# rvp-group/mad-icp

Hardware: NVIDIA H100
Metric: scans/sec (130k-pt scan vs 16-keyframe model) (higher is better)
Workload: dtype f64

## Files before the change

### mad_icp_b200/csrc/capi.cu

```cuda
#include <cooperative_groups.h>
#include <cuda_runtime.h>

#include <algorithm>
#include <cmath>
#include <cstdio>
#include <cstdlib>
#include <cstring>
#include <new>
#include <stdexcept>
#include <string>
#include <vector>

#include "../../include/madicp_b200_debug.h"
#include "ctx.hpp"
#include "device_kernels.cuh"

namespace madicp {

static thread_local std::string g_error;
void set_error(const std::string& msg) { g_error = msg; }

}

using namespace madicp;
// ... 792 lines not shown
  if (int rc = cloud_check(t, xyz_out, idx_out, fn)) return rc;
  const int64_t n = t->n_points;
  if (n == 0) return 0;
  madicp_ctx* c = t->ctx;
  MADICP_TRY
  CK(cudaSetDevice(c->device));
  if (size_t(n) > c->cap_cloud_out) {
    c->cap_cloud_out = 0;
    const size_t cap = size_t(n) + size_t(n) / 4 + 1024;
    CK(cudaHostAlloc(c->h_cloud_xyz.put(), cap * 3 * sizeof(double), cudaHostAllocMapped));
    CK(cudaHostAlloc(c->h_cloud_idx.put(), cap * sizeof(int64_t), cudaHostAllocMapped));
    c->cap_cloud_out = cap;
  }
  double* dx = nullptr;
  int64_t* di = nullptr;
  CK(cudaHostGetDevicePointer(reinterpret_cast<void**>(&dx), c->h_cloud_xyz, 0));
  CK(cudaHostGetDevicePointer(reinterpret_cast<void**>(&di), c->h_cloud_idx, 0));
  if (int rc = cloud_launch(t, X, xyz_out ? dx : nullptr, idx_out ? di : nullptr)) return rc;
  CK(cudaStreamSynchronize(c->stream));
  if (xyz_out) memcpy(xyz_out, c->h_cloud_xyz, size_t(n) * 3 * sizeof(double));
  if (idx_out) memcpy(idx_out, c->h_cloud_idx, size_t(n) * sizeof(int64_t));
  return n;
  MADICP_CATCH(fn)
}

int64_t madtree_gpu_cloud_dev(const madtree_gpu_t* t, const double X[12], double* xyz_out, int64_t* idx_out,
                              void* consumer_stream) {
  const char* fn = "madtree_gpu_cloud_dev";
  if (int rc = cloud_check(t, xyz_out, idx_out, fn)) return rc;
  madicp_ctx* c = t->ctx;
  CK(cudaSetDevice(c->device));
  if (xyz_out)
    if (int rc = madicp_check_device_ptr(c, xyz_out, 8, "madtree_gpu_cloud_dev (points)")) return rc;
  if (idx_out)
    if (int rc = madicp_check_device_ptr(c, idx_out, 8, "madtree_gpu_cloud_dev (indices)")) return rc;
  const int64_t n = t->n_points;
  if (n == 0) return 0;
  if (int rc = madicp_stream_wait(c, c->stream, consumer_stream)) return rc;
  if (int rc = cloud_launch(t, X, xyz_out, idx_out)) return rc;
  if (int rc = madicp_stream_wait(c, consumer_stream, c->stream)) return rc;
  return n;
}

int madtree_gpu_release_cloud(madtree_gpu_t* t) {
  if (!t) {
    set_error("madtree_gpu_release_cloud: null tree");
    return MADICP_ERR_INVALID;
  }
  t->cloud.reset();
  return MADICP_OK;
}

int madicp_put_keyframe_tree(madicp_ctx_t* c, int slot, const madtree_gpu_t* t, const double X[12]) {
  if (!c || !t || t->ctx != c || slot < 0 || slot >= c->max_keyframes || t->n_nodes < 1) {
    set_error("madicp_put_keyframe_tree: bad arguments (the tree must live on this context)");
    return MADICP_ERR_INVALID;
  }
  MADICP_TRY
  CK(cudaSetDevice(c->device));
  int rc = ensure_pool(c, size_t(t->n_nodes));
  if (rc) return rc;
  const double* X_dev = nullptr;
  if (X) {
    rc = stage_pose(c, X, &X_dev);
    if (rc) return rc;
  }
  CK(cudaMemcpyAsync(c->d_pool_lvl + size_t(slot) * (kMaxLevels + 1), t->lvl, size_t(t->n_levels + 1) * sizeof(int),
                     cudaMemcpyDeviceToDevice, c->stream));
  Slot& s = c->slots[slot];
  s.n_nodes = t->n_nodes;
  s.n_leaves = t->n_leaves;
  s.n_levels = t->n_levels;
  return build_slot(c, slot, t->recs, X_dev);
  MADICP_CATCH("madicp_put_keyframe_tree")
}

static int ensure_moving(madicp_ctx* c, int L) {
  if (size_t(L) <= c->cap_moving) return MADICP_OK;
  CK(cudaStreamSynchronize(c->stream));
  c->cap_moving = 0;
  const size_t cap = size_t(L) + size_t(L) / 4 + 1024;
  CK(cudaMalloc(c->d_moving.put(), cap * 3 * sizeof(double)));
  CK(cudaMalloc(c->d_mov4.put(), cap * sizeof(Moving4)));
  CK(cudaMalloc(c->d_step_matched.put(), cap));
  c->cap_moving = cap;
  return MADICP_OK;
}

static int prepare_moving(madicp_ctx* c) {
  if (!c->mov4_stale || c->L < 1) return MADICP_OK;
  k_prepare_moving<<<blocks_for(c->L), kStepBlock, 0, c->stream>>>(c->d_moving, c->L, c->P, c->d_mov4, nullptr, nullptr);
  c->launches++;
  CK(cudaGetLastError());
  c->mov4_stale = false;
  return MADICP_OK;
}

int madicp_set_moving(madicp_ctx_t* c, const double* means, int L) {
  if (!c || !means || L < 1 || size_t(L) > kMatchedCap) {
    set_error("madicp_set_moving: bad arguments (1 <= L <= 1048576)");
    return MADICP_ERR_INVALID;
  }
  CK(cudaSetDevice(c->device));
  int rc = ensure_moving(c, L);
  if (rc) return rc;
  CK(cudaMemcpyAsync(c->d_moving, means, size_t(L) * 3 * sizeof(double), cudaMemcpyHostToDevice, c->stream));
  c->L = L;
  c->mov4_stale = true;
  return prepare_moving(c);
}

int madicp_set_moving_tree(madicp_ctx_t* c, const madtree_gpu_t* t) {
  if (!c || !t || t->ctx != c || t->n_leaves < 1 || size_t(t->n_leaves) > kMatchedCap) {
    set_error("madicp_set_moving_tree: bad arguments (the tree must live on this context)");
    return MADICP_ERR_INVALID;
  }
  CK(cudaSetDevice(c->device));
  int rc = ensure_moving(c, t->n_leaves);
  if (rc) return rc;
  c->L = t->n_leaves;
  k_prepare_moving<<<blocks_for(c->L), kStepBlock, 0, c->stream>>>(c->d_moving, c->L, c->P, c->d_mov4, t->recs, t->leaf_of);
  c->launches++;
  CK(cudaGetLastError());
  c->mov4_stale = false;
  return MADICP_OK;
}

int madicp_get_moving(madicp_ctx_t* c, double* means_out, int cap) {
  if (!c || !means_out || c->L < 1 || cap < c->L) return MADICP_ERR_INVALID;
  CK(cudaSetDevice(c->device));
  CK(cudaMemcpyAsync(means_out, c->d_moving, size_t(c->L) * 3 * sizeof(double), cudaMemcpyDeviceToHost, c->stream));
  CK(cudaStreamSynchronize(c->stream));
  return c->L;
}

static int check_ready(madicp_ctx* c, const char* who) {
  if (!c) return MADICP_ERR_INVALID;
  if (c->L < 1 || !c->d_moving) {
    set_error(std::string(who) + ": no moving leaves (call madicp_set_moving first)");
    return MADICP_ERR_STATE;
  }
  if (int64_t(madicp_num_keyframes(c)) * int64_t(c->L) >= (int64_t(1) << 31)) {
    set_error(std::string(who) + ": keyframes x moving leaves must stay below 2^31 (32-bit item index)");
    return MADICP_ERR_INVALID;
  }
  if (madicp_num_keyframes(c) < 1 && c->world <= 1) {
    set_error(std::string(who) + ": no keyframe uploaded");
    return MADICP_ERR_STATE;
  }
  return MADICP_OK;
}

static int launch_search(madicp_ctx* c, const ModelView& mv, const double* d_X, bool want_ord) {
  const int64_t items = int64_t(mv.K) * c->L;
  int rc = ensure_items(c, size_t(items));
  if (rc) return rc;
  rc = prepare_moving(c);
  if (rc) return rc;
  k_search<<<grid_for(c, items), kStepBlock, 0, c->stream>>>(mv, c->d_mov4, c->L, d_X, c->d_hit,
                                                            want_ord ? c->d_ord.get() : nullptr);
  c->launches++;
  CK(cudaGetLastError());
  return MADICP_OK;
}

int madicp_search(madicp_ctx_t* c, const double X[12], int32_t* out) {
// ... 20 lines not shown
  if (rc) return rc;
  if (!X || !H || !b) return MADICP_ERR_INVALID;
  CK(cudaSetDevice(c->device));
  const ModelView mv = make_view(c);
  if (mv.K < 1) {
    set_error("madicp_linearize: no keyframe on this device");
    return MADICP_ERR_STATE;
  }
  memcpy(c->h_pinned, X, 12 * sizeof(double));
  CK(cudaMemcpyAsync(c->d_X, c->h_pinned, 12 * sizeof(double), cudaMemcpyHostToDevice, c->stream));
  rc = launch_search(c, mv, c->d_X, false);
  if (rc) return rc;
  CK(cudaMemsetAsync(c->d_state, 0, 16, c->stream));
  CK(cudaMemsetAsync(c->d_step_matched, 0, size_t(c->L), c->stream));
  const int64_t items = int64_t(mv.K) * c->L;
  const int grid = grid_for(c, items);
  k_linearize<<<grid, kStepBlock, 0, c->stream>>>(mv, c->d_mov4, c->L, c->d_X, c->P, c->d_hit, c->d_step_matched,
                                                 c->d_partial, c->d_state);
  c->launches++;
  CK(cudaGetLastError());
  CK(cudaMemcpyAsync(c->h_state, c->d_state, offsetof(GnState, X_trace), cudaMemcpyDeviceToHost, c->stream));
  if (matched) CK(cudaMemcpyAsync(c->h_matched, c->d_step_matched, size_t(c->L), cudaMemcpyDeviceToHost, c->stream));
  CK(cudaStreamSynchronize(c->stream));
  memcpy(H, c->h_state->H, sizeof(double) * 36);
  memcpy(b, c->h_state->b, sizeof(double) * 6);
  if (matched) memcpy(matched, c->h_matched, size_t(c->L));
  return MADICP_OK;
}

int madicp_solve_update(madicp_ctx_t* c, const double H[36], const double b[6], double X[12]) {
  if (!c || !H || !b || !X) return MADICP_ERR_INVALID;
  CK(cudaSetDevice(c->device));
  memcpy(c->h_pinned, X, 12 * sizeof(double));
  memcpy(c->h_pinned + 12, H, 36 * sizeof(double));
  memcpy(c->h_pinned + 48, b, 6 * sizeof(double));
  CK(cudaMemcpyAsync(c->d_X, c->h_pinned, 54 * sizeof(double), cudaMemcpyHostToDevice, c->stream));
  k_solve<<<1, 32, 0, c->stream>>>(c->d_X + 12, c->d_X + 48, c->d_X);
  c->launches++;
  CK(cudaGetLastError());
  CK(cudaMemcpyAsync(c->h_pinned, c->d_X, 12 * sizeof(double), cudaMemcpyDeviceToHost, c->stream));
  CK(cudaStreamSynchronize(c->stream));
  memcpy(X, c->h_pinned, 12 * sizeof(double));
  return MADICP_OK;
}

int madicp_debug_inv_det6(madicp_ctx_t* c, const double H[36], double* weight) {
  if (!c || !H || !weight) return MADICP_ERR_INVALID;
  CK(cudaSetDevice(c->device));
  memcpy(c->h_pinned + 12, H, 36 * sizeof(double));
  CK(cudaMemcpyAsync(c->d_X + 12, c->h_pinned + 12, 36 * sizeof(double), cudaMemcpyHostToDevice, c->stream));
  k_inv_det6<<<1, 32, 0, c->stream>>>(c->d_X + 12, c->d_X + 48);
  c->launches++;
  CK(cudaGetLastError());
  CK(cudaMemcpyAsync(c->h_pinned + 48, c->d_X + 48, sizeof(double), cudaMemcpyDeviceToHost, c->stream));
  CK(cudaStreamSynchronize(c->stream));
  *weight = c->h_pinned[48];
  return MADICP_OK;
}

static int register_enqueue(madicp_ctx* c, int iters, const double X0[12], int clear_from) {
  int rc = check_ready(c, "madicp_register");
  if (rc) return rc;
  if (!X0 || iters < 1 || iters > MADICP_MAX_ITERS) {
    set_error("madicp_register: bad arguments (1 <= iters <= 64 per launch)");
    return MADICP_ERR_INVALID;
  }
  CK(cudaSetDevice(c->device));
  rc = prepare_moving(c);
  if (rc) return rc;
  rc = pick_shape(c, int64_t(madicp_num_keyframes(c)) * c->L);
  if (rc) return rc;
  GnArgs A;
  A.model = make_view(c);
  A.P = c->P;
  A.peers.rank = c->rank;
  A.peers.world = c->world;
  A.peers.epoch_base = c->epoch;
  const int mb = int(c->call_seq & 1u);
  for (int r = 0; r < kMaxPeers; ++r) {
    A.peers.box[r] = (r < c->world) ? &c->peer_comm[r]->box : nullptr;
    A.peer_matched[r] = (r < c->world) ? c->peer_comm[r]->matched[mb] : nullptr;
  }
  A.moving = c->d_mov4;
  A.L = c->L;
  A.iters = iters;
  A.clear_from = clear_from;
  A.matched = c->d_comm->matched[mb];
  size_t map_bytes = 0;
  {
    const size_t per_cta = gn_map_bytes(unsigned(madicp_num_keyframes(c)), unsigned(c->L), unsigned(c->gn_grid));
    const size_t ctas = size_t(c->gn_grid / c->sm_count);
    auto bucket = [&](size_t dynamic) {
      const size_t bytes = ctas * (dynamic + c->gn_static_smem + 1024);
      const size_t kb[] = {8, 16, 32, 64, 100, 132, 164, 196, 228};
      for (size_t b : kb)
        if (bytes <= b * 1024) return b;
      return size_t(1 << 20);
    };
    if (per_cta && bucket(c->gn_smem + per_cta) == bucket(c->gn_smem)) map_bytes = per_cta;
  }
  A.map_in_smem = map_bytes ? 1 : 0;
  {
    const size_t stride =
        ((size_t(c->max_keyframes) * gn_share_bound(c->cap_moving, unsigned(c->gn_grid))) + 31) & ~size_t(31);
    const size_t need = stride * size_t(c->gn_grid);
    if (need > c->cap_memo) {
      CK(cudaStreamSynchronize(c->stream));
      c->cap_memo = 0;
      const size_t cap = need + need / 4;
      CK(cudaMalloc(c->d_memo_leaf.put(), cap * sizeof(int)));
      CK(cudaMalloc(c->d_memo_margin.put(), cap * sizeof(float)));
      CK(cudaMalloc(c->d_memo_ckpt.put(), cap * sizeof(unsigned)));
      CK(cudaMalloc(c->d_memo_ckpt_up.put(), cap * sizeof(float)));
      c->cap_memo = cap;
    }
    A.memo_leaf = c->d_memo_leaf;
    A.memo_margin = c->d_memo_margin;
    A.memo_ckpt = c->d_memo_ckpt;
    A.memo_ckpt_up = c->d_memo_ckpt_up;
    A.item_stride = int(stride);
    A.memo_mode = c->memo_mode;
    A.walk_buf = mb;
  }
  A.st = c->d_state;
  A.dbg = c->d_dbg;
  A.dbg_cta = c->d_dbg ? c->d_dbg_cta.get() : nullptr;
  c->epoch += uint32_t(iters);
  A.pose_epoch = c->pose_epoch;
  c->pose_epoch += uint32_t(iters);
  memcpy(A.X0, X0, 12 * sizeof(double));
  A.tiles = c->d_tiles;
  A.zero_next = c->d_comm->matched[mb ^ 1];
  A.zero_bytes = int((std::min(kMatchedCap, c->cap_moving) + 15) & ~size_t(15));
  void* args[] = {&A};
  CK(cudaLaunchCooperativeKernel(c->gn_kernel, dim3(c->gn_grid), dim3(c->gn_threads), args, c->gn_smem + map_bytes, c->stream));
  c->launches++;
  c->last_iters = iters;
  c->call_seq++;
  return MADICP_OK;
}

int madicp_register_async(madicp_ctx_t* c, int iters, const double X0[12]) {
  return register_enqueue(c, iters, X0, iters - 1);
}
int madicp_register_partial_async(madicp_ctx_t* c, int iters, const double X0[12]) {
  return register_enqueue(c, iters, X0, 0);
}

int madicp_register_fetch_weight(madicp_ctx_t* c, double X[12], double H[36], double b[6], uint8_t* matched, int* n_matched,
                                 double* weight) {
  if (!c || c->last_iters < 1) {
    set_error("madicp_register_fetch: nothing was enqueued");
    return MADICP_ERR_STATE;
  }
  CK(cudaSetDevice(c->device));
  CK(cudaMemcpyAsync(c->h_state, c->d_state, offsetof(GnState, X_trace), cudaMemcpyDeviceToHost, c->stream));
  if (matched)
    CK(cudaMemcpyAsync(c->h_matched, c->d_comm->matched[(c->call_seq - 1u) & 1u], size_t(c->L), cudaMemcpyDeviceToHost,
                       c->stream));
  CK(cudaStreamSynchronize(c->stream));
  if (c->h_state->error) {
    set_error("madicp_register: a peer GPU never delivered its H/b tile (rank down, or no matching registration enqueued there)");
    CK(cudaMemsetAsync(&c->d_state->error, 0, sizeof(int), c->stream));
    return MADICP_ERR_COMM;
  }
  if (X) memcpy(X, c->h_state->X_out, 12 * sizeof(double));
  if (H) memcpy(H, c->h_state->H, 36 * sizeof(double));
  if (b) memcpy(b, c->h_state->b, 6 * sizeof(double));
  if (matched) memcpy(matched, c->h_matched, size_t(c->L));
  if (n_matched) *n_matched = c->h_state->n_matched;
  if (weight) *weight = c->h_state->weight;
  return MADICP_OK;
}
int madicp_register_fetch(madicp_ctx_t* c, double X[12], double H[36], double b[6], uint8_t* matched, int* n_matched) {
  return madicp_register_fetch_weight(c, X, H, b, matched, n_matched, nullptr);
}

int madicp_register(madicp_ctx_t* c, int iters, double X[12], double H[36], double b[6], uint8_t* matched,
                    int* n_matched) {
  if (!c || !X || iters < 0) {
    set_error("madicp_register: bad arguments");
    return MADICP_ERR_INVALID;
  }
  if (iters == 0) {
    if (H) memset(H, 0, 36 * sizeof(double));
    if (b) memset(b, 0, 6 * sizeof(double));
    if (matched && c->L > 0) memset(matched, 0, size_t(c->L));
    if (n_matched) *n_matched = 0;
    return MADICP_OK;
  }
  int left = iters;
  while (left > MADICP_MAX_ITERS) {
    int rc = register_enqueue(c, MADICP_MAX_ITERS, X, MADICP_MAX_ITERS);
    if (rc) return rc;
    rc = madicp_register_fetch(c, X, nullptr, nullptr, nullptr, nullptr);
    if (rc) return rc;
    left -= MADICP_MAX_ITERS;
  }
  int rc = register_enqueue(c, left, X, left - 1);
  if (rc) return rc;
  return madicp_register_fetch(c, X, H, b, matched, n_matched);
}
// ... 271 lines not shown
```

### mad_icp_b200/csrc/ctx.hpp

```cpp
#pragma once
#include <cuda_runtime.h>

#include <atomic>
#include <memory>
#include <mutex>
#include <new>
#include <stdexcept>
#include <string>
#include <vector>

#include "cuda_owned.hpp"
#include "kernels.cuh"

namespace madicp {
void set_error(const std::string& msg);

constexpr int kMaxLevels = 4096;
struct Slot {
  int n_nodes = 0, n_leaves = 0, n_levels = 0;
};
constexpr size_t kMatchedCap = size_t(1) << 20;

struct CommBlock {
  Mailbox box;
  unsigned char matched[2][kMatchedCap];
};

struct CloudBuf {
  size_t cap = 0;
  DevPtr<double> xyz;
  DevPtr<int32_t> idx;
};
}

struct madicp_ctx;

struct madtree_gpu {
  madicp_ctx* ctx = nullptr;
  madtree_rec_t* recs = nullptr;
  int* lvl = nullptr;
  int* leaf_of = nullptr;
  size_t cap_nodes = 0;
  void* block = nullptr;
  int n_nodes = 0, n_leaves = 0, n_levels = 0;
  std::vector<int> h_lvl;
  double* full = nullptr;
  int64_t n_points = 0;
  uint64_t build_seq = 0;
  std::shared_ptr<madicp::CloudBuf> cloud;
  int64_t cloud_off = 0;
};

struct madicp_ctx {
  ~madicp_ctx();
  int device = 0;
  int max_keyframes = 0;
  madicp::Stream own_stream;
  cudaStream_t stream = nullptr;
  int sm_count = 0;
  std::vector<madicp::Slot> slots;
  size_t pool_cap = 0;
  madicp::DevPtr<madtree_rec_t> d_pool_recs;
  madicp::DevPtr<int> d_pool_child0;
  madicp::DevPtr<int> d_pool_rec_of;
  madicp::DevPtr<int> d_pool_lvl;
  size_t quad_cap = 0;
  madicp::DevPtr<madicp::QuadRec> d_quad;
  madicp::DevPtr<double> d_pool_ww;
  static constexpr int kXformRing = 64;
  madicp::DevPtr<double> d_xform;
  madicp::HostPtr<double> h_xform;
  madicp::HostPtr<int> h_lvl;
  madicp::Event xform_done[kXformRing];
  uint32_t xform_seq = 0;
  static constexpr int kGatherRing = 8;
  madicp::HostPtr<madicp::LeafGather> h_gather;
  madicp::DevPtr<madicp::LeafGather> d_gather;
  size_t cap_gather = 0;
  madicp::Event gather_done[kGatherRing];
  uint32_t gather_seq = 0;
  madicp::DevPtr<double> d_leaves;
  madicp::HostPtr<double> h_leaves;
  size_t cap_leaves = 0;
  std::vector<madtree_gpu*> tree_cache;
  std::vector<madicp::DevPtr<void>> tree_slabs;
  madicp::Event tree_free_ev;
  madicp::Event xstream_ev;
  std::mutex tree_mu;
  bool keep_cloud = false;
  std::vector<madicp::CloudBuf*> cloud_cache;
  std::mutex cloud_mu;
  madicp::HostPtr<int64_t> h_cloud_idx;
  madicp::HostPtr<double> h_cloud_xyz;
  size_t cap_cloud_out = 0;
  void* build_state = nullptr;
  void* plan_state = nullptr;
  madicp::DevPtr<long long> d_dbg_cta;
  madicp::IcpParams P{0.2, 0.31622776601683794, 0.02};
  madicp::DevPtr<double> d_moving;
  madicp::DevPtr<madicp::Moving4> d_mov4;
  bool mov4_stale = true;
  madicp::DevPtr<unsigned char> d_step_matched;
  int L = 0;
  size_t cap_moving = 0;
  uint32_t call_seq = 0;
  madicp::DevPtr<int> d_hit;
  madicp::DevPtr<int> d_ord;
  size_t cap_items = 0;
  madicp::DevPtr<double> d_cloud_q;
  madicp::DevPtr<int> d_cloud_o;
  size_t cap_cloud = 0;
  madicp::DevPtr<double> d_partial;
  madicp::DevPtr<madicp::LLCell> d_tiles;
  size_t cap_partial = 0;
  madicp::DevPtr<int> d_memo_leaf;
  madicp::DevPtr<float> d_memo_margin;
  madicp::DevPtr<unsigned> d_memo_ckpt;
  madicp::DevPtr<float> d_memo_ckpt_up;
  size_t cap_memo = 0;
  int memo_mode = 2;
  madicp::DevPtr<madicp::GnState> d_state;
  madicp::DevPtr<double> d_X;
  madicp::DevPtr<madicp::CommBlock> d_comm;
  madicp::HostPtr<double> h_pinned;
  madicp::HostPtr<madicp::GnState> h_state;
  madicp::HostPtr<unsigned char> h_matched;
  int gn_grid = 0;
  bool gn_auto = true;
  int gn_threads = 1024;
  const void* gn_kernel = nullptr;
  size_t gn_smem = 0;
  size_t gn_static_smem = 0;
  static constexpr int kNumAutoShapes = 5;
  static constexpr int kAutoShapes[kNumAutoShapes] = {768, 896, 704, 640, 512};
  double pass_cost[kNumAutoShapes] = {4935.0, 6195.0, 5060.0, 4925.0, 4165.0};
  bool calibrated = false;
  int last_iters = 0;
  madicp::DevPtr<long long> d_dbg;
  std::atomic<int64_t> launches{0};
  int rank = 0, world = 1;
  madicp::CommBlock* peer_comm[madicp::kMaxPeers] = {};
  uint32_t epoch = 0;
  uint32_t pose_epoch = 1;
};

#define CK(call)                                                                                   \
  do {                                                                                             \
    cudaError_t e_ = (call);                                                                       \
    if (e_ != cudaSuccess) {                                                                       \
      madicp::set_error(std::string(#call) + ": " + cudaGetErrorString(e_));                       \
      return MADICP_ERR_CUDA;                                                                      \
    }                                                                                              \
  } while (0)

#define MADICP_TRY try {
#define MADICP_CATCH(who)                                          \
  }                                                                \
  catch (const std::bad_alloc&) {                                  \
    madicp::set_error(std::string(who) + ": out of host memory");  \
    return MADICP_ERR_NOMEM;                                       \
  }                                                                \
  catch (const std::exception& e_) {                               \
    madicp::set_error(std::string(who) + ": " + e_.what());        \
    return MADICP_ERR_INVALID;                                     \
  }

int madicp_tree_alloc(madicp_ctx* c, size_t cap_nodes, madtree_gpu** out);
int madicp_cloud_alloc(madicp_ctx* c, size_t n, std::shared_ptr<madicp::CloudBuf>* out);
int madicp_check_device_ptr(madicp_ctx* c, const void* p, int align, const char* fn);
int madicp_stream_wait(madicp_ctx* c, void* waiter, void* signaller);
void madicp_gpu_build_release(madicp_ctx* c);
```

### mad_icp_b200/csrc/device_kernels.cuh

```cuda
#pragma once
#include "gn_partition.h"
#include "kernels.cuh"

namespace madicp {


__device__ __forceinline__ int depth_of(const int* __restrict__ lvl, int n_levels, int i) {
  int lo = 0, hi = n_levels;
  while (hi - lo > 1) {
    const int mid = (lo + hi) >> 1;
    if (__ldg(lvl + mid) <= i) lo = mid; else hi = mid;
  }
  return lo;
}

__global__ void __launch_bounds__(kStepBlock)
k_slot_ingest(const madtree_rec_t* src, madtree_rec_t* dst, int n, const double* __restrict__ Xp,
              const int* __restrict__ lvl, int n_levels, int* __restrict__ flag) {
  const int i = blockIdx.x * kStepBlock + threadIdx.x;
  if (i >= n) return;
  Rec r = load_rec_plain(src + i);
  const int npts = src[i].num_points;
  int f = 0;
  if (r.link >= 0 && (depth_of(lvl, n_levels, i) & 1) == 0)
// ... 277 lines not shown
  }
}

__global__ void __launch_bounds__(kStepBlock)
k_search_cloud(const __grid_constant__ ModelView model, int root, const char* __restrict__ q, int64_t n, int64_t q_stride,
               int q_is_f32, int* __restrict__ ordinals, double* __restrict__ points, double* __restrict__ normals,
               double* __restrict__ dists) {
  for (int64_t i = int64_t(blockIdx.x) * kStepBlock + threadIdx.x; i < n; i += int64_t(gridDim.x) * kStepBlock) {
    const char* r = q + i * q_stride;
    double qx, qy, qz;
    if (q_is_f32) {
      const float* f = reinterpret_cast<const float*>(r);
      qx = double(__ldg(f)); qy = double(__ldg(f + 1)); qz = double(__ldg(f + 2));
    } else {
      const double* d = reinterpret_cast<const double*>(r);
      qx = __ldg(d); qy = __ldg(d + 1); qz = __ldg(d + 2);
    }
    double ww;
    const Rec f = load_rec(model.recs + descend(model, root, qx, qy, qz, ww));
    if (ordinals) ordinals[i] = -1 - f.link;
    if (points) {
      points[3 * i] = f.mx; points[3 * i + 1] = f.my; points[3 * i + 2] = f.mz;
    }
    if (normals) {
      normals[3 * i] = f.dx; normals[3 * i + 1] = f.dy; normals[3 * i + 2] = f.dz;
    }
    if (dists) dists[i] = norm3(qx - f.mx, qy - f.my, qz - f.mz);
  }
}


template <int THREADS>
__device__ __forceinline__ void peer_allreduce(const PeerView& pv, uint32_t epoch, double* s_tot,
                                               double (*s_peer)[kAcc], int* error) {
  const int slot = int(epoch & 1u);
  for (int idx = threadIdx.x; idx < pv.world * kAcc; idx += THREADS) {
    const int r = idx / kAcc, i = idx - r * kAcc;
    const double v = s_tot[i];
    const uint32_t lo = uint32_t(__double2loint(v)), hi = uint32_t(__double2hiint(v));
    LLCell* dst = &pv.box[r]->cell[slot][pv.rank][i];
    asm volatile("st.volatile.global.v4.u32 [%0], {%1,%2,%3,%4};" ::"l"(dst), "r"(lo), "r"(epoch), "r"(hi), "r"(epoch)
                 : "memory");
  }
  for (int idx = threadIdx.x; idx < pv.world * kAcc; idx += THREADS) {
    const int r = idx / kAcc, i = idx - r * kAcc;
    const LLCell* src = &pv.box[pv.rank]->cell[slot][r][i];
    uint32_t lo, f0, hi, f1, spins = 0;
    do {
      asm volatile("ld.volatile.global.v4.u32 {%0,%1,%2,%3}, [%4];" : "=r"(lo), "=r"(f0), "=r"(hi), "=r"(f1) : "l"(src)
                   : "memory");
      if (++spins == (1u << 26)) {
        *error = 1;
        break;
      }
    } while (f0 != epoch || f1 != epoch);
    s_peer[r][i] = __hiloint2double(int(hi), int(lo));
  }
  __syncthreads();
  if (threadIdx.x < kAcc) {
    double s = s_peer[0][threadIdx.x];
    for (int r = 1; r < pv.world; ++r) s += s_peer[r][threadIdx.x];
    s_tot[threadIdx.x] = s;
  }
  __syncthreads();
}

struct GnArgs {
  ModelView model;
  IcpParams P;
  PeerView peers;
  const Moving4* moving;
  int L;
  int iters;
  int clear_from;
  unsigned char* matched;
  unsigned char* peer_matched[kMaxPeers];
  LLCell* tiles;
  double X0[12];
  unsigned char* zero_next;
  int zero_bytes;
  GnState* st;
  int map_in_smem;
  uint32_t pose_epoch;
  int* memo_leaf;
  float* memo_margin;
  unsigned* memo_ckpt;
  float* memo_ckpt_up;
  int item_stride;
  int walk_buf;
  int memo_mode;
  long long* dbg;
  long long* dbg_cta;
};
#ifndef MADICP_CKPT_TAU_SCALE
#define MADICP_CKPT_TAU_SCALE 1.0
#endif
__device__ __forceinline__ float ckpt_tau(int it, double moved, double ball) {
  return __double2float_ru(MADICP_CKPT_TAU_SCALE * (it == 0 ? ball : moved));
}

__device__ __forceinline__ long long global_ns() {
  long long t;
  asm volatile("mov.u64 %0, %%globaltimer;" : "=l"(t));
  return t;
}

template <int THREADS, int CTAS>
__global__ void __launch_bounds__(THREADS, CTAS)
k_gn_loop(const __grid_constant__ GnArgs A) {
  constexpr int WARPS = THREADS / 32;
  extern __shared__ __align__(16) double s_dyn[];
  double* s_stage_all = s_dyn;
  double(*s_red)[64] = reinterpret_cast<double(*)[64]>(s_dyn);
  double(*s_peer)[kAcc] = reinterpret_cast<double(*)[kAcc]>(s_dyn + WARPS * 64);
  static_assert(WARPS * 64 + kMaxPeers * kAcc <= WARPS * kStageTile, "scratch must fit in the staging tiles");
  __shared__ double s_tot[kAcc];
  __shared__ double s_b[6];
  __shared__ double s_X[12], s_Xp[12];
  __shared__ int s_qn, s_rn;
  __shared__ int s_count[WARPS];
  __shared__ unsigned s_plo[kGnPieces], s_pn[kGnPieces];
  GnState* st = A.st;
  const unsigned L = unsigned(A.L);
  const unsigned total = unsigned(A.model.K) * L;
  const bool multi = A.peers.world > 1;
  const unsigned lane = threadIdx.x & 31;
  const unsigned warp = threadIdx.x >> 5;
  double* stage = s_stage_all + warp * kStageTile;
  constexpr unsigned kPieces = kGnPieces;
  unsigned n_b = 0;
#pragma unroll
  for (unsigned p = 0; p < kPieces; ++p) {
    unsigned lo, n;
    gn_stretch(L, gridDim.x, blockIdx.x, p, lo, n);
    if (threadIdx.x == 0) {
      s_plo[p] = lo;
      s_pn[p] = n;
    }
    n_b += n;
  }
  __syncthreads();
  const unsigned t_total = unsigned(A.model.K) * n_b;
  (void) total;
  auto item_of = [&](unsigned t0, unsigned& k, unsigned& q) {
    k = t0 / n_b;
    q = t0 - k * n_b + lane;
    while (q >= n_b) {
      q -= n_b;
      ++k;
    }
    const unsigned j = q;
    q = s_plo[kPieces - 1] + (j - (n_b - s_pn[kPieces - 1]));
    unsigned acc = 0;
#pragma unroll
    for (unsigned p = 0; p + 1 < kPieces; ++p) {
      const unsigned n = s_pn[p];
      if (j >= acc && j < acc + n) q = s_plo[p] + (j - acc);
      acc += n;
    }
  };
  unsigned* s_map = A.map_in_smem ? reinterpret_cast<unsigned*>(s_dyn + WARPS * kStageTile) : nullptr;
  if (s_map) {
    for (unsigned t0 = warp * 32; t0 < t_total; t0 += THREADS) {
      unsigned k, q;
      item_of(t0, k, q);
      s_map[t0 + lane] = (k << 26) | q;
    }
    __syncwarp();
  }

  for (int i = (blockIdx.x * THREADS + threadIdx.x) * 16; i < A.zero_bytes; i += gridDim.x * THREADS * 16)
    *reinterpret_cast<uint4*>(A.zero_next + i) = make_uint4(0, 0, 0, 0);
  if (blockIdx.x == 0 && threadIdx.x < MADICP_MAX_ITERS) {
    st->walked[A.walk_buf ^ 1][threadIdx.x] = 0;
    st->walk_recs[A.walk_buf ^ 1][threadIdx.x] = 0;
  }
  const unsigned memo0 = blockIdx.x * unsigned(A.item_stride);
  auto item_at = [&](unsigned t0, unsigned& k, unsigned& q) {
    if (s_map) {
      const unsigned pk = s_map[t0 + lane];
      k = pk >> 26;
      q = pk & 0x3ffffffu;
    } else {
      item_of(t0, k, q);
    }
  };

  for (int it = 0; it < A.iters; ++it) {
    if (threadIdx.x < 12) {
      double x;
      if (it == 0) {
        x = A.X0[threadIdx.x];
      } else {
        const uint32_t ep = A.pose_epoch + uint32_t(it);
        uint32_t lo, hi, f0, f1;
        do {
          ll_load(&st->X_ll[threadIdx.x], lo, f0, hi, f1);
        } while (f0 != ep || f1 != ep);
        x = __hiloint2double(int(hi), int(lo));
      }
      s_Xp[threadIdx.x] = s_X[threadIdx.x];
      s_X[threadIdx.x] = x;
      if (it == 0 && blockIdx.x == 0) st->X_trace[threadIdx.x] = x;
    }
    if (threadIdx.x == 32) s_qn = 0;
    if (threadIdx.x == 33) s_rn = 0;
    __syncthreads();
    const bool last_round = (it == A.iters - 1);
    double c0 = 0.0, c1 = 0.0;
    long long t_begin = 0;
    if (A.dbg && threadIdx.x == 0) t_begin = clock64();
    const size_t dbg_plane = size_t(MADICP_MAX_ITERS) * gridDim.x, dbg_at = size_t(it) * gridDim.x + blockIdx.x;
    if (A.dbg_cta && threadIdx.x == 0) A.dbg_cta[dbg_plane + dbg_at] = global_ns();

    int n_walked = 0, n_recs = 0;
    for (unsigned t0 = warp * 32; t0 < t_total; t0 += THREADS) {
      unsigned k, q;
      item_at(t0, k, q);
      double v[kStage];
#pragma unroll
      for (int i = 0; i < kStage; ++i) v[i] = 0.0;
      const unsigned t = t0 + lane;
      if (t < t_total) {
        const Moving4 m = load_moving(A.moving + q);
        double mx, my, mz;
        iso_apply(s_X, m.px, m.py, m.pz, mx, my, mz);
        int leaf = -1;
        unsigned start = 0;
        float prefix = __int_as_float(0x7f800000);
        double moved = 0.0;
        if (it > 0 && A.memo_mode) {
          const float have = A.memo_margin[memo0 + t];
          const int last = A.memo_leaf[memo0 + t];
          unsigned ck = 0;
          float ck_up = 0.0f;
          if (A.memo_mode == 2) {
            ck = A.memo_ckpt[memo0 + t];
            ck_up = A.memo_ckpt_up[memo0 + t];
          }
          double bx, by, bz;
          iso_apply(s_Xp, m.px, m.py, m.pz, bx, by, bz);
          const double dx = mx - bx, dy = my - by, dz = mz - bz;
          moved = 1.0001 * sqrt(dx * dx + dy * dy + dz * dz) + 1e-9 + 1e-12 * (fabs(mx) + fabs(my) + fabs(mz));
          const double left = double(have) - moved;
          if (left > 0.0) {
            A.memo_margin[memo0 + t] = __double2float_rd(left);
            leaf = last;
          } else if (ck != 0) {
            const double ck_left = __dsub_rd(__dadd_rd(double(have), double(ck_up)), moved);
            if (ck_left > 0.0) {
              start = ck;
              prefix = __double2float_rd(ck_left);
            }
          }
        }
        if (leaf < 0) {
          double ww_walk;
          const float tau = ckpt_tau(it, moved, m.ball);
          float margin = prefix, ck_margin = 0.0f;
          unsigned ckpt = start;
          leaf = A.memo_mode ? descend_t<true>(A.model, int(k), mx, my, mz, ww_walk, margin, ckpt, ck_margin, tau, n_recs)
                             : descend_t<false>(A.model, int(k), mx, my, mz, ww_walk, margin, ckpt, ck_margin, tau, n_recs);
          if (A.memo_mode) {
            A.memo_leaf[memo0 + t] = leaf;
            A.memo_margin[memo0 + t] = margin;
          }
          if (A.memo_mode == 2) {
            A.memo_ckpt[memo0 + t] = ckpt;
            A.memo_ckpt_up[memo0 + t] = __fsub_rd(ck_margin, margin);
          }
          ++n_walked;
        }
        const double ww = __ldg(A.model.ww + leaf);
        const Rec f = load_rec(A.model.recs + leaf);
        const Moving4 m2 = load_moving(A.moving + q);
        if (linearize_one(s_X, A.P.rho_ker_sqrt, m2, mx, my, mz, f, ww, v) && it >= A.clear_from) {
          if (multi) {
            for (int r = 0; r < A.peers.world; ++r) A.peer_matched[r][q] = 1;
          } else {
            A.matched[q] = 1;
          }
        }
      }
      warp_accumulate(stage, v, c0, c1);
    }
    n_walked = __reduce_add_sync(0xffffffffu, n_walked);
    n_recs = __reduce_add_sync(0xffffffffu, n_recs);
    if (lane == 0 && n_walked) {
      atomicAdd(&s_qn, n_walked);
      atomicAdd(&s_rn, n_recs);
    }
    if (A.dbg && threadIdx.x == 0 && blockIdx.x == 0) A.dbg[it * 8 + 0] = clock64() - t_begin;
    if (A.dbg_cta) {
      __syncthreads();
      if (threadIdx.x == 0) {
        A.dbg_cta[dbg_at] = clock64() - t_begin;
        A.dbg_cta[2 * dbg_plane + dbg_at] = global_ns();
      }
      if (threadIdx.x == 0 && blockIdx.x == 0) A.dbg[it * 8 + 5] = s_qn;
    }
    __syncthreads();
    if (threadIdx.x == 0 && s_qn) {
      atomicAdd(&st->walked[A.walk_buf][it], s_qn);
      atomicAdd(&st->walk_recs[A.walk_buf][it], (unsigned long long) s_rn);
    }
    const uint32_t ep_round = A.pose_epoch + uint32_t(it);
    block_reduce_publish<WARPS>(c0, c1, s_red, A.tiles + size_t(blockIdx.x) * kAcc, ep_round,
                                 it >= A.clear_from, multi);
    if (A.dbg_cta && threadIdx.x == 0) A.dbg_cta[3 * dbg_plane + dbg_at] = global_ns();
    if (blockIdx.x == 0) {
      long long t0 = 0, t1 = 0, t2 = 0;
      if (A.dbg && threadIdx.x == 0) t0 = clock64();
      fold_tiles<THREADS>(A.tiles, gridDim.x, ep_round, s_red, s_tot,
                          (A.dbg_cta && gridDim.x >= 16) ? A.dbg_cta + 4 * dbg_plane + size_t(it) * gridDim.x : nullptr);
      if (A.dbg && threadIdx.x == 0) {
        t1 = clock64();
        A.dbg[it * 8 + 1] = t1 - t_begin;
        A.dbg[it * 8 + 2] = t1 - t0;
        A.dbg[it * 8 + 6] = global_ns();
      }
      if (multi) {
        if (last_round) __threadfence_system();
        peer_allreduce<THREADS>(A.peers, A.peers.epoch_base + uint32_t(it) + 1u, s_tot, s_peer, &st->error);
        if (last_round) __threadfence_system();
      }
      if (last_round) {
        __threadfence();
        int c = 0;
        {
          const uint4* m16 = reinterpret_cast<const uint4*>(A.matched);
          for (int q = threadIdx.x; q < (A.L + 15) / 16; q += THREADS) {
            const uint4 w = __ldcv(m16 + q);
            c += __popc(w.x) + __popc(w.y) + __popc(w.z) + __popc(w.w);
          }
        }
        for (int off = 16; off > 0; off >>= 1) c += __shfl_down_sync(0xffffffffu, c, off);
        if (lane == 0) s_count[warp] = c;
      }
      if (threadIdx.x < 6) s_b[threadIdx.x] = s_tot[threadIdx.x * 8 + 6];
      __syncthreads();
      if (last_round && threadIdx.x >= 32) {
        if (threadIdx.x == 32) unpack_Hb(s_tot, st->H, st->b);
        if (threadIdx.x == 64) st->weight = inv_det6_dev(s_tot, 8);
        if (threadIdx.x == 96) {
          int c = 0;
          for (int w2 = 0; w2 < WARPS; ++w2) c += s_count[w2];
          st->n_matched = c;
        }
      }
      if (threadIdx.x == 0) {
        if (A.dbg) t2 = clock64();
        double Xn[12];
        gn_update_pose(s_tot, 8, s_b, s_X, Xn);
        if (!last_round) {
          const uint32_t ep = ep_round + 1u;
#pragma unroll
          for (int i = 0; i < 12; ++i) ll_store(&st->X_ll[i], Xn[i], ep);
        }
#pragma unroll
// ... 22 lines not shown
```

### mad_icp_b200/csrc/kernels.cuh

```cuda
#pragma once
#include <cuda_runtime.h>
#include <stdint.h>

#include "../../include/madicp_b200.h"
#include "arith.h"
#include "solve6.h"

namespace madicp {

constexpr int kMaxSlots = 64;
constexpr int kStepBlock = 256;
constexpr int kAcc = 48;
constexpr int kStage = 8;
constexpr int kStageItems = 16;
constexpr int kStagePitch = 20;
constexpr int kStageTile = kStage * kStagePitch;
constexpr int kMaxPeers = 16;
constexpr int kMailboxSlots = 2;

struct __align__(16) FastRec {
  float dx, dy, dz, c;
};
static_assert(sizeof(FastRec) == 16, "FastRec must be one 128-bit load");

constexpr float kBoundC = 1.0e-6f;

struct __align__(32) QuadRec {
  FastRec p0, p1, p2;
  int bfs0;
  int child0;
  int pad[2];
};
static_assert(sizeof(QuadRec) == 64, "QuadRec must be four 128-bit loads");

struct ModelView {
  const madtree_rec_t* recs;
  const QuadRec* quad;
  const double* ww;
  int broot[kMaxSlots];
  int qroot[kMaxSlots];
  int K;
};
constexpr unsigned kLeafMarker = 0x7fc0beefu;

struct IcpParams {
  double min_ball, rho_ker_sqrt, b_ratio;
};

struct __align__(32) Moving4 {
  double px, py, pz, ball;
};

struct LeafGather {
  const madtree_rec_t* recs;
  const int* leaf_of;
  int out, n_leaves, has_pose, pad;
  double X[12];
};

struct CloudOut {
  const double* xyz;
  const int32_t* idx;
  long long n;
  int has_pose, pad;
  double X[12];
};

struct __align__(16) LLCell {
  uint32_t lo, flag_lo, hi, flag_hi;
};

__device__ __forceinline__ void ll_store(LLCell* p, double v, uint32_t epoch) {
  asm volatile("st.volatile.global.v4.u32 [%0], {%1,%2,%3,%4};" ::"l"(p), "r"(uint32_t(__double2loint(v))), "r"(epoch),
               "r"(uint32_t(__double2hiint(v))), "r"(epoch) : "memory");
}
__device__ __forceinline__ void ll_load(const LLCell* p, uint32_t& lo, uint32_t& f0, uint32_t& hi, uint32_t& f1) {
  asm volatile("ld.volatile.global.v4.u32 {%0,%1,%2,%3}, [%4];" : "=r"(lo), "=r"(f0), "=r"(hi), "=r"(f1) : "l"(p) : "memory");
}

struct GnState {
  int ticket;
  int clear_from;
  int n_matched;
  int error;
  double X_in[12];
  double X_out[12];
  double H[36];
  double b[6];
  double weight;
  double X_trace[(MADICP_MAX_ITERS + 1) * 12];
  int walked[2][MADICP_MAX_ITERS];
  unsigned long long walk_recs[2][MADICP_MAX_ITERS];
  LLCell X_ll[12];
};

struct Mailbox {
  LLCell cell[kMailboxSlots][kMaxPeers][kAcc];
};

struct PeerView {
  Mailbox* box[kMaxPeers];
  int rank, world;
  uint32_t epoch_base;
};

struct Rec {
  double mx, my, mz, dx, dy, dz, bbox0;
  int link;
};

__device__ __forceinline__ void ld_nc_f64x2(const void* p, double& a, double& b) {
  asm volatile("ld.global.nc.v2.f64 {%0,%1}, [%2];" : "=d"(a), "=d"(b) : "l"(p));
}
__device__ __forceinline__ void ld_nc_f32x4(const void* p, float& a, float& b, float& c, float& d) {
  asm volatile("ld.global.nc.v4.f32 {%0,%1,%2,%3}, [%4];" : "=f"(a), "=f"(b), "=f"(c), "=f"(d) : "l"(p));
}
__device__ __forceinline__ void ld_nc_s32x4(const void* p, int& a, int& b, int& c, int& d) {
  asm volatile("ld.global.nc.v4.s32 {%0,%1,%2,%3}, [%4];" : "=r"(a), "=r"(b), "=r"(c), "=r"(d) : "l"(p));
}

__device__ __forceinline__ Rec load_rec(const madtree_rec_t* p) {
  double a0, a1, a2, a3, b0, b1, b2, b3;
  const char* q = reinterpret_cast<const char*>(p);
  ld_nc_f64x2(q, a0, a1);
  ld_nc_f64x2(q + 16, a2, a3);
  ld_nc_f64x2(q + 32, b0, b1);
  ld_nc_f64x2(q + 48, b2, b3);
  Rec r;
  r.mx = a0; r.my = a1; r.mz = a2; r.dx = a3; r.dy = b0; r.dz = b1; r.bbox0 = b2;
  r.link = __double2loint(b3);
  return r;
}

__device__ __forceinline__ Rec load_rec_plain(const madtree_rec_t* p) {
// ... 329 lines not shown
```

Baseline: 5363.

## Precompute per-point transformed positions and cumulative motion once per GN round

```diff
diff --git a/mad_icp_b200/csrc/capi.cu b/mad_icp_b200/csrc/capi.cu
--- a/mad_icp_b200/csrc/capi.cu
+++ b/mad_icp_b200/csrc/capi.cu
@@ -898,6 +898,7 @@
   const size_t cap = size_t(L) + size_t(L) / 4 + 1024;
   CK(cudaMalloc(c->d_moving.put(), cap * 3 * sizeof(double)));
   CK(cudaMalloc(c->d_mov4.put(), cap * sizeof(Moving4)));
+  CK(cudaMalloc(c->d_leaf_round.put(), cap * sizeof(LeafRound)));
   CK(cudaMalloc(c->d_step_matched.put(), cap));
   c->cap_moving = cap;
   return MADICP_OK;
@@ -1084,6 +1085,7 @@
     A.peer_matched[r] = (r < c->world) ? c->peer_comm[r]->matched[mb] : nullptr;
   }
   A.moving = c->d_mov4;
+  A.leaf_round = c->d_leaf_round;
   A.L = c->L;
   A.iters = iters;
   A.clear_from = clear_from;
@@ -1111,15 +1113,15 @@
       c->cap_memo = 0;
       const size_t cap = need + need / 4;
       CK(cudaMalloc(c->d_memo_leaf.put(), cap * sizeof(int)));
-      CK(cudaMalloc(c->d_memo_margin.put(), cap * sizeof(float)));
+      CK(cudaMalloc(c->d_memo_budget.put(), cap * sizeof(float)));
       CK(cudaMalloc(c->d_memo_ckpt.put(), cap * sizeof(unsigned)));
-      CK(cudaMalloc(c->d_memo_ckpt_up.put(), cap * sizeof(float)));
+      CK(cudaMalloc(c->d_memo_ck_budget.put(), cap * sizeof(float)));
       c->cap_memo = cap;
     }
     A.memo_leaf = c->d_memo_leaf;
-    A.memo_margin = c->d_memo_margin;
+    A.memo_budget = c->d_memo_budget;
     A.memo_ckpt = c->d_memo_ckpt;
-    A.memo_ckpt_up = c->d_memo_ckpt_up;
+    A.memo_ck_budget = c->d_memo_ck_budget;
     A.item_stride = int(stride);
     A.memo_mode = c->memo_mode;
     A.walk_buf = mb;
diff --git a/mad_icp_b200/csrc/ctx.hpp b/mad_icp_b200/csrc/ctx.hpp
--- a/mad_icp_b200/csrc/ctx.hpp
+++ b/mad_icp_b200/csrc/ctx.hpp
@@ -99,6 +99,7 @@
   madicp::IcpParams P{0.2, 0.31622776601683794, 0.02};
   madicp::DevPtr<double> d_moving;
   madicp::DevPtr<madicp::Moving4> d_mov4;
+  madicp::DevPtr<madicp::LeafRound> d_leaf_round;
   bool mov4_stale = true;
   madicp::DevPtr<unsigned char> d_step_matched;
   int L = 0;
@@ -114,9 +115,9 @@
   madicp::DevPtr<madicp::LLCell> d_tiles;
   size_t cap_partial = 0;
   madicp::DevPtr<int> d_memo_leaf;
-  madicp::DevPtr<float> d_memo_margin;
+  madicp::DevPtr<float> d_memo_budget;
   madicp::DevPtr<unsigned> d_memo_ckpt;
-  madicp::DevPtr<float> d_memo_ckpt_up;
+  madicp::DevPtr<float> d_memo_ck_budget;
   size_t cap_memo = 0;
   int memo_mode = 2;
   madicp::DevPtr<madicp::GnState> d_state;
diff --git a/mad_icp_b200/csrc/device_kernels.cuh b/mad_icp_b200/csrc/device_kernels.cuh
--- a/mad_icp_b200/csrc/device_kernels.cuh
+++ b/mad_icp_b200/csrc/device_kernels.cuh
@@ -383,10 +383,11 @@
   GnState* st;
   int map_in_smem;
   uint32_t pose_epoch;
+  LeafRound* leaf_round;
   int* memo_leaf;
-  float* memo_margin;
+  float* memo_budget;
   unsigned* memo_ckpt;
-  float* memo_ckpt_up;
+  float* memo_ck_budget;
   int item_stride;
   int walk_buf;
   int memo_mode;
@@ -417,7 +418,7 @@
   static_assert(WARPS * 64 + kMaxPeers * kAcc <= WARPS * kStageTile, "scratch must fit in the staging tiles");
   __shared__ double s_tot[kAcc];
   __shared__ double s_b[6];
-  __shared__ double s_X[12], s_Xp[12];
+  __shared__ double s_X[12];
   __shared__ int s_qn, s_rn;
   __shared__ int s_count[WARPS];
   __shared__ unsigned s_plo[kGnPieces], s_pn[kGnPieces];
@@ -443,15 +444,8 @@
   __syncthreads();
   const unsigned t_total = unsigned(A.model.K) * n_b;
   (void) total;
-  auto item_of = [&](unsigned t0, unsigned& k, unsigned& q) {
-    k = t0 / n_b;
-    q = t0 - k * n_b + lane;
-    while (q >= n_b) {
-      q -= n_b;
-      ++k;
-    }
-    const unsigned j = q;
-    q = s_plo[kPieces - 1] + (j - (n_b - s_pn[kPieces - 1]));
+  auto leaf_at = [&](unsigned j) {
+    unsigned q = s_plo[kPieces - 1] + (j - (n_b - s_pn[kPieces - 1]));
     unsigned acc = 0;
 #pragma unroll
     for (unsigned p = 0; p + 1 < kPieces; ++p) {
@@ -459,6 +453,16 @@
       if (j >= acc && j < acc + n) q = s_plo[p] + (j - acc);
       acc += n;
     }
+    return q;
+  };
+  auto item_of = [&](unsigned t0, unsigned& k, unsigned& q) {
+    k = t0 / n_b;
+    unsigned j = t0 - k * n_b + lane;
+    while (j >= n_b) {
+      j -= n_b;
+      ++k;
+    }
+    q = leaf_at(j);
   };
   unsigned* s_map = A.map_in_smem ? reinterpret_cast<unsigned*>(s_dyn + WARPS * kStageTile) : nullptr;
   if (s_map) {
@@ -488,6 +492,13 @@
   };
 
   for (int it = 0; it < A.iters; ++it) {
+    for (unsigned j = threadIdx.x; j < n_b; j += THREADS) {
+      const unsigned q = leaf_at(j);
+      const char* mp = reinterpret_cast<const char*>(A.moving + q);
+      const char* ep = reinterpret_cast<const char*>(A.leaf_round + q);
+      asm volatile("prefetch.global.L1 [%0];" ::"l"(mp));
+      if (it > 0) asm volatile("prefetch.global.L1 [%0]; prefetch.global.L1 [%1];" ::"l"(ep), "l"(ep + sizeof(LeafRound) - 8));
+    }
     if (threadIdx.x < 12) {
       double x;
       if (it == 0) {
@@ -500,12 +511,30 @@
         } while (f0 != ep || f1 != ep);
         x = __hiloint2double(int(hi), int(lo));
       }
-      s_Xp[threadIdx.x] = s_X[threadIdx.x];
       s_X[threadIdx.x] = x;
       if (it == 0 && blockIdx.x == 0) st->X_trace[threadIdx.x] = x;
     }
     if (threadIdx.x == 32) s_qn = 0;
     if (threadIdx.x == 33) s_rn = 0;
+    __syncthreads();
+    for (unsigned j = threadIdx.x; j < n_b; j += THREADS) {
+      const unsigned q = leaf_at(j);
+      const Moving4 m = load_moving(A.moving + q);
+      LeafRound* e = A.leaf_round + q;
+      LeafRound r;
+      iso_apply(s_X, m.px, m.py, m.pz, r.mx, r.my, r.mz);
+      double moved = 0.0;
+      r.c_hi = r.c_lo = 0.0;
+      if (it > 0) {
+        const double dx = r.mx - e->mx, dy = r.my - e->my, dz = r.mz - e->mz;
+        moved = 1.0001 * sqrt(dx * dx + dy * dy + dz * dz) + 1e-9 + 1e-12 * (fabs(r.mx) + fabs(r.my) + fabs(r.mz));
+        r.c_hi = __dadd_ru(e->c_hi, moved);
+        r.c_lo = __dadd_rd(e->c_lo, moved);
+      }
+      r.tau = ckpt_tau(it, moved, m.ball);
+      r.pad = 0.0f;
+      *e = r;
+    }
     __syncthreads();
     const bool last_round = (it == A.iters - 1);
     double c0 = 0.0, c1 = 0.0;
@@ -523,59 +552,49 @@
       for (int i = 0; i < kStage; ++i) v[i] = 0.0;
       const unsigned t = t0 + lane;
       if (t < t_total) {
-        const Moving4 m = load_moving(A.moving + q);
-        double mx, my, mz;
-        iso_apply(s_X, m.px, m.py, m.pz, mx, my, mz);
+        const LeafRound* e = A.leaf_round + q;
+        const double2 e0 = reinterpret_cast<const double2*>(e)[0], e1 = reinterpret_cast<const double2*>(e)[1];
+        const double mx = e0.x, my = e0.y, mz = e1.x, c_hi = e1.y;
         int leaf = -1;
         unsigned start = 0;
         float prefix = __int_as_float(0x7f800000);
-        double moved = 0.0;
         if (it > 0 && A.memo_mode) {
-          const float have = A.memo_margin[memo0 + t];
+          const float budget = A.memo_budget[memo0 + t];
           const int last = A.memo_leaf[memo0 + t];
           unsigned ck = 0;
-          float ck_up = 0.0f;
+          float ck_budget = 0.0f;
           if (A.memo_mode == 2) {
             ck = A.memo_ckpt[memo0 + t];
-            ck_up = A.memo_ckpt_up[memo0 + t];
+            ck_budget = A.memo_ck_budget[memo0 + t];
           }
-          double bx, by, bz;
-          iso_apply(s_Xp, m.px, m.py, m.pz, bx, by, bz);
-          const double dx = mx - bx, dy = my - by, dz = mz - bz;
-          moved = 1.0001 * sqrt(dx * dx + dy * dy + dz * dz) + 1e-9 + 1e-12 * (fabs(mx) + fabs(my) + fabs(mz));
-          const double left = double(have) - moved;
-          if (left > 0.0) {
-            A.memo_margin[memo0 + t] = __double2float_rd(left);
+          if (double(budget) > c_hi) {
             leaf = last;
-          } else if (ck != 0) {
-            const double ck_left = __dsub_rd(__dadd_rd(double(have), double(ck_up)), moved);
-            if (ck_left > 0.0) {
-              start = ck;
-              prefix = __double2float_rd(ck_left);
-            }
+          } else if (ck != 0 && double(ck_budget) > c_hi) {
+            start = ck;
+            prefix = __double2float_rd(__dsub_rd(double(ck_budget), c_hi));
           }
         }
         if (leaf < 0) {
           double ww_walk;
-          const float tau = ckpt_tau(it, moved, m.ball);
           float margin = prefix, ck_margin = 0.0f;
           unsigned ckpt = start;
-          leaf = A.memo_mode ? descend_t<true>(A.model, int(k), mx, my, mz, ww_walk, margin, ckpt, ck_margin, tau, n_recs)
-                             : descend_t<false>(A.model, int(k), mx, my, mz, ww_walk, margin, ckpt, ck_margin, tau, n_recs);
+          leaf = A.memo_mode ? descend_t<true>(A.model, int(k), mx, my, mz, ww_walk, margin, ckpt, ck_margin, e->tau, n_recs)
+                             : descend_t<false>(A.model, int(k), mx, my, mz, ww_walk, margin, ckpt, ck_margin, 0.0f, n_recs);
           if (A.memo_mode) {
+            const double c_lo = e->c_lo;
             A.memo_leaf[memo0 + t] = leaf;
-            A.memo_margin[memo0 + t] = margin;
-          }
-          if (A.memo_mode == 2) {
-            A.memo_ckpt[memo0 + t] = ckpt;
-            A.memo_ckpt_up[memo0 + t] = __fsub_rd(ck_margin, margin);
+            A.memo_budget[memo0 + t] = __double2float_rd(__dadd_rd(double(margin), c_lo));
+            if (A.memo_mode == 2) {
+              A.memo_ckpt[memo0 + t] = ckpt;
+              A.memo_ck_budget[memo0 + t] = __double2float_rd(__dadd_rd(double(ck_margin), c_lo));
+            }
           }
           ++n_walked;
         }
         const double ww = __ldg(A.model.ww + leaf);
         const Rec f = load_rec(A.model.recs + leaf);
-        const Moving4 m2 = load_moving(A.moving + q);
-        if (linearize_one(s_X, A.P.rho_ker_sqrt, m2, mx, my, mz, f, ww, v) && it >= A.clear_from) {
+        const Moving4 m = load_moving(A.moving + q);
+        if (linearize_one(s_X, A.P.rho_ker_sqrt, m, mx, my, mz, f, ww, v) && it >= A.clear_from) {
           if (multi) {
             for (int r = 0; r < A.peers.world; ++r) A.peer_matched[r][q] = 1;
           } else {
diff --git a/mad_icp_b200/csrc/kernels.cuh b/mad_icp_b200/csrc/kernels.cuh
--- a/mad_icp_b200/csrc/kernels.cuh
+++ b/mad_icp_b200/csrc/kernels.cuh
@@ -50,6 +50,15 @@
 struct __align__(32) Moving4 {
   double px, py, pz, ball;
 };
+
+struct __align__(16) LeafRound {
+  double mx, my, mz;
+  double c_hi;
+  double c_lo;
+  float tau;
+  float pad;
+};
+static_assert(sizeof(LeafRound) == 48, "LeafRound: three 128-bit words");
 
 struct LeafGather {
   const madtree_rec_t* recs;
```

After: 5374 (median of 6 runs). About the same (+0.2%).
